# uniio/ivf-hnsw

Measured on AMD Instinct MI355X. Metric: queries/sec @ Recall@1, SIFT1B PQ16 nprobe=32; ADC scan HBM GB/s vs peak, higher is better.
Workload: dtype f32

## Files before the change

### ivf-hnsw_amd/csrc/capi_upload.cpp

```cpp
#include "capi_internal.h"

namespace {

int check_desc(const ivfhnsw_ivf_desc *d, bool need_lists)
{
    if (!d)
        return fail(IVFHNSW_ERR_INVALID, "null descriptor");
    if (d->d == 0 || d->nc == 0 || d->code_size == 0)
        return fail(IVFHNSW_ERR_INVALID, "d, nc and code_size must be positive");
    if (d->code_size % 4)
        return fail(IVFHNSW_ERR_INVALID, "code_size %zu is not a multiple of 4 (IndexIVF_HNSW.cpp:805)", d->code_size);
    if (d->code_size * 1024 > kScanDynLdsMax)
        return fail(IVFHNSW_ERR_INVALID, "code_size %zu: the query's table (1 KB per code byte) must fit %zu KB of LDS",
                    d->code_size, kScanDynLdsMax / 1024);
    if (d->d % d->code_size)
        return fail(IVFHNSW_ERR_INVALID, "d %zu is not a multiple of code_size %zu", d->d, d->code_size);
    if (d->d / d->code_size > 64)
        return fail(IVFHNSW_ERR_INVALID, "sub-vector dimension %zu > 64 unsupported", d->d / d->code_size);
    if (d->nc >= 0xffffffffull)
        return fail(IVFHNSW_ERR_INVALID, "nc too large");
    if (!d->offsets || !d->centroid_norms || !d->pq_centroids || !d->norm_table)
        return fail(IVFHNSW_ERR_INVALID, "offsets, centroid_norms, pq_centroids and norm_table are required");
    if (need_lists && d->offsets[d->nc] != 0 && (!d->ids || !d->codes || !d->norm_codes))
        return fail(IVFHNSW_ERR_INVALID, "ids, codes and norm_codes are required");
// ... 397 lines not shown
        link_counts = counts_u.data();
        links = links_u.data();
        unique = true;
    }
    if ((rc = upload(h->q_counts, link_counts, n)))
        return rc;
    if ((rc = upload(h->q_links, links, n * maxM * sizeof(uint32_t))))
        return rc;
    if ((rc = upload(h->q_vectors, vectors, n * d * sizeof(float))))
        return rc;
    h->gr.n = (uint32_t)n;
    h->gr.d = (int)d;
    h->gr.maxM = (int)maxM;
    h->gr.enterpoint = enterpoint;
    h->gr.counts = h->q_counts.as<uint8_t>();
    h->gr.links = h->q_links.as<uint32_t>();
    h->gr.vectors = h->q_vectors.as<float>();
    {
        static const int merge = [] {
            const char *e = getenv("IVFHNSW_WALK_MERGE");
            return (e && atoi(e) == 0) ? 0 : 1;
        }();
        h->gr.merge_admissions = merge;
        h->gr.skip_padding = 1;
    }
    {
        static const int late_knob = [] {
            const char *e = getenv("IVFHNSW_WALK_LATE_VISIT");
            return e ? (atoi(e) != 0 ? 1 : 0) : -1;
        }();
        const bool late = late_knob < 0 ? n > 255u * 1008u : late_knob == 1;
        h->gr.links_unique = (unique && late) ? 1 : 0;
    }
    h->gr.fat = nullptr;
    h->gr.qrows = nullptr;
    h->gr.nbrows = nullptr;
    h->gr.nbnorms = nullptr;
    h->gr.links_c = nullptr;
    h->gr.nb_rows = 0;
    h->gr.q_lo = 0.f;
    h->gr.q_step = 1.f;
    h->gr.q_errc = 0.f;
    if ((rc = build_byte_rows(h, n, d, vectors)))
        return rc;
    if ((rc = build_neighbour_rows(h)))
        return rc;
    h->has_graph = true;
// ... 96 lines not shown
```

### ivf-hnsw_amd/csrc/ivfhnsw_kernels.h

```cpp
#pragma once

#include <hip/hip_runtime.h>
#include <mutex>
#include <stdint.h>

#include "scan_dispatch.h"
#include "sweep_plan_math.h"
#include "update_math.h"

namespace ivfhnsw_gpu_impl {

struct DynLdsState {
    std::mutex m;
    size_t raised[64] = {};
};
inline hipError_t raise_dyn_lds(const void *kern, size_t bytes, DynLdsState &st)
{
    int dev = 0;
    hipError_t e = hipGetDevice(&dev);
    if (e != hipSuccess)
        return e;
    if (dev < 0 || dev >= 64)
        return hipFuncSetAttribute(kern, hipFuncAttributeMaxDynamicSharedMemorySize, (int)bytes);
    std::lock_guard<std::mutex> lk(st.m);
// ... 75 lines not shown
    int nsubc;
    const float *alphas;
    const uint32_t *nn_idx;
    const uint32_t *sub_sizes;
    const float *inter_dists;
    int dedupe;
};

struct GraphTables {
    uint32_t n;
    int d, maxM;
    uint32_t enterpoint;
    const uint8_t *counts;
    const uint32_t *links;
    const float *vectors;
    const uint8_t *qrows;
    float q_lo, q_step, q_errc;
    const uint8_t *nbrows;
    const uint32_t *nbnorms;
    const uint32_t *links_c;
    int nb_rows;
    const float *fat;
    int visited_clean;
    int skip_padding;
    int merge_admissions;
    int links_unique;
};

hipError_t launch_opq(hipStream_t s, const float *At, const float *x, float *y, int nq, int d);
hipError_t launch_lut(hipStream_t s, const IvfTables &t, const float *xq, float *luts, int nq, const PlanHdr *hdr = nullptr);
hipError_t launch_plan_ivf(hipStream_t s, const IvfTables &t, const uint32_t *coarse_ids, const float *coarse_dists,
                           int nprobe, uint64_t max_codes, const PlanView &p, uint64_t *keys, int k);
hipError_t launch_plan_lut(hipStream_t s, const IvfTables &t, const float *xq, const uint32_t *coarse_ids,
                           const float *coarse_dists, int nprobe, uint64_t max_codes, const PlanView &p, uint64_t *keys,
                           int k, float *luts);
hipError_t launch_plan_grouping(hipStream_t s, const IvfTables &t, const GroupTables &g, const GraphTables &gr,
                                const float *xq, const uint32_t *coarse_ids, const float *coarse_dists, int nprobe,
                                uint64_t max_codes, int do_pruning, const PlanView &p, uint64_t *keys, int k,
                                float *qsd_scratch);
struct ScanOut {
    uint64_t *stream = nullptr;
    uint32_t *stream_len = nullptr;
    uint32_t stream_cap = 0;
    float *sel_dist = nullptr;
    int64_t *sel_labels = nullptr;
};
hipError_t launch_scan(hipStream_t s, const IvfTables &t, const float *luts, const PlanView &p, int k, int nsplit,
// ... 194 lines not shown
```

### ivf-hnsw_amd/csrc/kernels_hnsw.hip

```cpp
#include "ivfhnsw_kernels.h"
#include "device_common.h"
#include "walk_set.h"

#include <float.h>
#include <stdio.h>
#include <stdlib.h>

namespace ivfhnsw_gpu_impl {

constexpr int vis_buckets(int minw, int tagw = 8)
{
    return minw <= 4 ? (tagw == 10 ? 1040 : 1008) : minw == 5 ? 768 : minw <= 7 ? 640 : 384;
}

template <int TAGW> struct VisFields {
    static constexpr int cntw = TAGW == 8 ? 8 : TAGW == 10 ? 14 : 16;
    static constexpr int cshift = 64 - cntw;
    static constexpr int slots = cshift / TAGW;
    static constexpr unsigned long long ones()
    {
        unsigned long long o = 0;
        for (int i = 0; i < slots; i++)
            o |= 1ull << (TAGW * i);
        return o;
    }
};

template <int TAGW, int NB>
__device__ __forceinline__ bool visit_test_and_set(uint32_t id, unsigned long long *vt, uint32_t *bm, bool &used_bitmap)
// ... 85 lines not shown
                    const float t1 = qv.y - (float)((ws[c] >> 8) & 0xffu);
                    const float t2 = qv.z - (float)((ws[c] >> 16) & 0xffu);
                    const float t3 = qv.w - (float)(ws[c] >> 24);
                    a0 = fmaf(t0, t0, a0);
                    a1 = fmaf(t1, t1, a1);
                    a2 = fmaf(t2, t2, a2);
                    a3 = fmaf(t3, t3, a3);
                }
            }
        }
    }
    return (a0 + a1) + (a2 + a3);
}

__device__ __forceinline__ unsigned long long walk_stamp()
{
    __builtin_amdgcn_sched_barrier(0);
    const unsigned long long t = __builtin_amdgcn_s_memtime();
    __builtin_amdgcn_s_waitcnt(0xC07F);
    __builtin_amdgcn_sched_barrier(0);
    return t;
}

template <int NCH, int MINW, int TAGW, int FMODE, bool STAMPS = false, bool SPILL = false>
__global__ __launch_bounds__(64, MINW) void hnsw_walk_kernel(GraphTables g, const float *__restrict__ xq, int nq, int nprobe,
                                                       int ef, uint32_t *__restrict__ coarse_ids,
                                                       float *__restrict__ coarse_dists,
                                                       uint32_t *__restrict__ visited, size_t vwords,
                                                       uint32_t *__restrict__ status, uint32_t *__restrict__ next_query,
                                                       uint32_t *__restrict__ redo_hdr, uint32_t *__restrict__ redo_list,
                                                       uint32_t *__restrict__ tail_bitmaps = nullptr,
                                                       unsigned long long *__restrict__ stamp_out = nullptr)
{
    extern __shared__ __attribute__((aligned(16))) unsigned char smem[];
    float *s_q = reinterpret_cast<float *>(smem);
    float *s_qp = s_q + g.d;
    const int dp = FMODE == 1 ? g.d : 0;
    uint32_t *s_q8 = reinterpret_cast<uint32_t *>(s_qp + dp);
    unsigned long long *tail = reinterpret_cast<unsigned long long *>(smem + (size_t)(g.d + dp) * sizeof(float) + 512);
    constexpr int NB = vis_buckets(MINW, TAGW);
    unsigned long long st_acc[9] = {0, 0, 0, 0, 0, 0}, st_t = 0;
    const int merge_extra = (NCH <= 4 && ef + 8 > kTailCap) ? ef + 8 - kTailCap : 0;
    unsigned long long *vt = tail + kTailCap + merge_extra;
    constexpr bool LDSVIS = TAGW != 0;

    const int lane = threadIdx.x;
    const int judged_row = 8 * (((lane >> 2) & 1) * 2 + (lane & 1)) + (lane >> 3);
    const bool merge_on = g.merge_admissions != 0;
    constexpr bool prefilter = FMODE != 0;
    constexpr bool inline_rows = FMODE >= 2;
    constexpr bool ROWNORMS = FMODE == 3;
    constexpr bool CK = FMODE >= 2;
    auto enc_id = [](uint32_t id, uint32_t c) { return CK ? (id << 7) | c : id; };
    auto dec_id = [](uint32_t e) { return CK ? e >> 7 : e; };
    uint32_t *bm = visited + (size_t)blockIdx.x * vwords;
    TailSpill spill;
    spill.bm = SPILL ? tail_bitmaps + (size_t)blockIdx.x * vwords : nullptr;
    spill.hi = -1;
    spill.count = 0;
    bool bitmap_dirty = !(LDSVIS && g.visited_clean);
    bool redo_ran = false;

    for (;;) {
        int q = 0;
        if constexpr (SPILL) {
            if (lane == 0) {
                const uint32_t i = atomicAdd(&redo_hdr[1], 1u);
                q = i < redo_hdr[0] ? (int)redo_list[i] : nq;
            }
        } else {
            if (lane == 0)
                q = (int)atomicAdd(next_query, 1u);
        }
        q = __builtin_amdgcn_readfirstlane(q);
        if (q >= nq)
            break;
        redo_ran = true;
        if (STAMPS)
            st_t = walk_stamp();

        if (!LDSVIS || bitmap_dirty) {
            uint4 *bm4 = reinterpret_cast<uint4 *>(bm);
            const size_t v4 = vwords / 4;
            for (size_t w = lane; w < v4; w += 64)
                bm4[w] = make_uint4(0u, 0u, 0u, 0u);
            bitmap_dirty = false;
        }
        if (LDSVIS)
            for (int w = lane; w < NB; w += 64)
                vt[w] = 0ull;
        __syncthreads();
        float qp_sq = 0.f;
        for (int i = lane; i < g.d; i += 64) {
            const float v = xq[(size_t)q * g.d + i];
            s_q[i] = v;
            if (prefilter) {
                const float vp = __fdiv_rn(__fsub_rn(v, g.q_lo), g.q_step);
                if (!inline_rows)
                    s_qp[i] = vp;
                qp_sq = fmaf(vp, vp, qp_sq);
            }
        }
        __syncthreads();
        constexpr bool QREG = MINW <= 4;
        float q_reg[QREG ? 16 : 1];
        if constexpr (QREG) {
#pragma unroll
            for (int i = 0; i < 16; i++)
                q_reg[i] = (g.d == 128 || g.d == 96) && 8 * i < g.d ? s_q[8 * i + (lane & 7)] : 0.f;
        }
        float pf_slack = 0.f, pf_slack_q = 0.f, pf_bonus = 0.f;
        int q16_w = 0;
        int x_const = 0;
        bool x_any = false;
        bool x_hi = false;
        uint4 qp_h = make_uint4(0u, 0u, 0u, 0u), qp_l = qp_h, qp_x = qp_h;
        if (prefilter) {
#pragma unroll
            for (int off = 32; off > 0; off >>= 1)
                qp_sq += __shfl_xor(qp_sq, off, 64);
            pf_slack = __uint_as_float(__builtin_amdgcn_readfirstlane(__float_as_uint(g.q_errc + 3.9e-6f * sqrtf(qp_sq))));
            if (inline_rows) {
                float dq_sq = 0.f, bonus = 0.f;
                int s_hh = 0, s_hl = 0, s_ll = 0, s_xh = 0, s_xl = 0;
                if (lane < 32) {
                    uint32_t wh = 0, wl = 0, wxl = 0, wxh = 0;
#pragma unroll
                    for (int b = 0; b < 4; b++) {
                        const int comp = 4 * lane + b;
                        const float vp = comp < g.d ? __fdiv_rn(__fsub_rn(s_q[comp], g.q_lo), g.q_step) : 0.f;
                        const float fh = fminf(255.f, fmaxf(0.f, floorf(vp)));
                        const float fl = fminf(255.f, fmaxf(0.f, rintf((vp - fh) * 256.f)));
                        const float qin = fh + fl * 0.00390625f;
                        const bool below = vp < 0.f, above = vp >= 256.f;
                        const float e = (below || above) ? 0.f : vp - qin;
                        dq_sq = fmaf(e, e, dq_sq);
                        const float out = (below || above) ? fabsf(vp - qin) : 0.f;
                        bonus = fmaf(out, out, bonus);
                        const int x = (int)fminf(255.f, floorf(2.f * out));
                        const int hi = (int)fh, lo = (int)fl;
                        s_hh += hi * hi;
                        s_hl += hi * lo;
                        s_ll += lo * lo;
                        wh |= (uint32_t)hi << (8 * b);
                        wl |= (uint32_t)lo << (8 * b);
                        if (below)
                            wxl |= (uint32_t)x << (8 * b);
                        if (above)
                            wxh |= (uint32_t)x << (8 * b);
                        s_xl += below ? x : 0;
                        s_xh += above ? x : 0;
                    }
                    s_q8[lane] = wh;
// ... 14 lines not shown
                s_xl = __builtin_amdgcn_readfirstlane(s_xl);
                s_xh = __builtin_amdgcn_readfirstlane(s_xh);
                q16_w = __builtin_amdgcn_readfirstlane(128 * s_hh + s_hl + (s_ll >> 9));
                x_any = (s_xl | s_xh) != 0;
                x_hi = s_xh != 0;
                x_const = 255 * s_xh;
                pf_slack_q = __uint_as_float(__builtin_amdgcn_readfirstlane(__float_as_uint(1.001f * sqrtf(dq_sq))));
                pf_bonus = __uint_as_float(__builtin_amdgcn_readfirstlane(__float_as_uint(0.999f * bonus)));
                __syncthreads();
                qp_h = *reinterpret_cast<const uint4 *>(s_q8 + 4 * (lane & 7));
                qp_l = *reinterpret_cast<const uint4 *>(s_q8 + 32 + 4 * (lane & 7));
                qp_x = *reinterpret_cast<const uint4 *>(s_q8 + 64 + 4 * (lane & 7));
            }
        }

        RSet<NCH> R;
#pragma unroll
        for (int cc = 0; cc < NCH; cc++)
            R.r[cc] = ~0ull;
        int n = 1;
        int ntail = 0;
        uint32_t tail_db = 0;
        {
            const float d0 = l2_ref_order_quad(g.vectors + (size_t)g.enterpoint * g.d, s_q, g.d, lane & 3);
            bool ub = false;
            if (lane == 0) {
                R.r[0] = mk_key(d0, enc_id(g.enterpoint, CK ? (uint32_t)g.counts[g.enterpoint] : 0u));
                (void)visit_test_and_set<TAGW, NB>(g.enterpoint, vt, bm, ub);
            }
            __syncthreads();
        }
        bool used_bitmap = false;
        bool pend = false, pend_any = false, pend_full = false;
        uint32_t pend_id = 0;
        if (STAMPS) {
            const unsigned long long t = walk_stamp();
            st_acc[4] += t - st_t;
            st_t = t;
        }

        for (;;) {
            const int first = R.first_unexpanded(n, lane);
            int pick = -1;
            int pick_tail = -1;
            uint32_t pick_id = 0;
            if (first >= 0) {
                const unsigned long long kfirst = R.get(first);
                const uint32_t db = key_dist_bits(kfirst);
                pick = first;
                pick_id = key_id(kfirst);
                if (first + 1 < n && key_dist_bits(R.get(first + 1)) == db) {
                    pick = R.last_unexpanded_with(db, first, n, lane);
                    pick_id = key_id(R.get(pick));
                }
                if (ntail > 0 && db == key_dist_bits(R.get(n - 1))) {
                    if (SPILL && spill.count > 0) {
                        const uint32_t sid = spill.peek_max(lane);
                        const uint32_t senc = enc_id(sid, CK ? (uint32_t)g.counts[sid] : 0u);
                        if (senc > pick_id) {
                            pick_id = senc;
                            pick_tail = kTailCap;
                        }
                    } else {
                        for (int t = 0; t < ntail; t++)
                            if (key_id(tail[t]) > pick_id) {
                                pick_id = key_id(tail[t]);
                                pick_tail = t;
                            }
                    }
                    if (pick_tail >= 0)
                        pick = -1;
                }
            } else if (SPILL && spill.count > 0) {
                const uint32_t sid = spill.peek_max(lane);
                pick_id = enc_id(sid, CK ? (uint32_t)g.counts[sid] : 0u);
                pick_tail = kTailCap;
            } else if (ntail > 0) {
                pick_tail = 0;
                pick_id = key_id(tail[0]);
                for (int t = 1; t < ntail; t++)
                    if (key_id(tail[t]) > pick_id) {
                        pick_id = key_id(tail[t]);
                        pick_tail = t;
                    }
            } else {
                break;
            }
            if (pick >= 0) {
                R.mark_expanded(pick, lane);
            } else if (SPILL && pick_tail == kTailCap) {
                spill.remove(dec_id(pick_id), lane);
                ntail--;
            } else {
                __syncthreads();
                if (lane == 0)
                    tail[pick_tail] = tail[ntail - 1];
                ntail--;
                __syncthreads();
            }

            if (STAMPS) {
                const unsigned long long t = walk_stamp();
                st_acc[0] += t - st_t;
                st_t = t;
                st_acc[5] += 1;
            }
            const uint32_t node = dec_id(pick_id);
            int cnt;
            uint32_t nb = 0, nb_enc = 0;
            if constexpr (CK) {
                cnt = (int)(pick_id & 127u);
                if (lane < g.maxM) {
                    const uint32_t raw = g.links_c[(size_t)node * g.maxM + lane];
                    nb = raw & 0xffffffu;
                    nb_enc = (nb << 7) | (raw >> 24);
                }
            } else {
                cnt = g.counts[node];
                if (lane < g.maxM)
                    nb = g.links[(size_t)node * g.maxM + lane];
                nb_enc = nb;
            }
            const bool filter_now = prefilter && n == ef;
            uint4 nw[4] = {};
            uint32_t row_rr = 0;
            if (filter_now && inline_rows) {
                if constexpr (CK) {
                    const uint4 *nbr = reinterpret_cast<const uint4 *>(g.nbrows + (size_t)node * g.nb_rows * 128) + (lane & 7);
                    const int last = max(cnt - 1, 0);
#pragma unroll
                    for (int i = 0; i < 4; i++)
                        if (8 * i < cnt)
                            nw[i] = nbr[min(8 * i + (lane >> 3), last) * 8];
                } else {
                    const uint4 *nbr = reinterpret_cast<const uint4 *>(g.nbrows + (size_t)node * g.nb_rows * 128) + lane;
#pragma unroll
                    for (int i = 0; i < 4; i++)
                        nw[i] = nbr[i * 64];
                }
                if constexpr (ROWNORMS)
                    row_rr = g.nbnorms[(size_t)node * g.nb_rows + judged_row];
            }
            constexpr bool LATE = FMODE == 3 && LDSVIS;
            const bool filter_first = LATE && filter_now;
            bool fresh = false, seen = false, full_now = false;
            if constexpr (LATE) {
                if (pend_any) {
                    if (pend)
                        visit_insert_absent<TAGW, NB>(pend_id, pend_full, vt, bm, used_bitmap);
                    pend_any = false;
                }
                if (lane < cnt) {
                    if (filter_first)
                        seen = visit_lookup<TAGW, NB>(nb, vt, bm, full_now);
                    else
                        fresh = visit_test_and_set<TAGW, NB>(nb, vt, bm, used_bitmap);
                }
            } else {
                if (lane < cnt)
                    fresh = visit_test_and_set<TAGW, NB>(nb, vt, bm, used_bitmap);
            }
            unsigned long long mask = __ballot(fresh);
            int nfresh = __popcll(mask);
            const unsigned long long last_now = R.get(n - 1);
            if (filter_now && inline_rows) {
                if (filter_first)
                    fresh = lane < cnt && !seen;
                const float worst = __uint_as_float(key_dist_bits(last_now));
                const uint32_t qh[4] = {qp_h.x, qp_h.y, qp_h.z, qp_h.w}, ql[4] = {qp_l.x, qp_l.y, qp_l.z, qp_l.w};
                const uint32_t xl[4] = {qp_x.x, qp_x.y, qp_x.z, qp_x.w};
                uint32_t xh[4] = {0u, 0u, 0u, 0u};
                if (x_hi) {
                    const uint4 b = *reinterpret_cast<const uint4 *>(s_q8 + 96 + 4 * (lane & 7));
                    xh[0] = b.x, xh[1] = b.y, xh[2] = b.z, xh[3] = b.w;
                }
                const int cnt_s = __builtin_amdgcn_readfirstlane(cnt);
                for (int rb = 0;;) {
                    int S[4], X[4];
#pragma unroll
                    for (int i = 0; i < 4; i++) {
                        if ((CK || g.skip_padding) && rb + 8 * i >= cnt_s) {
                            S[i] = 0;
                            X[i] = 0;
                            continue;
                        }
                        const uint32_t ws[4] = {nw[i].x, nw[i].y, nw[i].z, nw[i].w};
                        uint32_t hr = 0, rr = 0;
#pragma unroll
                        for (int c = 0; c < 4; c++) {
                            hr = __builtin_amdgcn_udot4(qh[c], ws[c], hr, false);
                            if constexpr (!ROWNORMS)
                                rr = __builtin_amdgcn_udot4(ws[c], ws[c], rr, false);
                        }
                        uint32_t lr = hr << 8;
#pragma unroll
                        for (int c = 0; c < 4; c++)
                            lr = __builtin_amdgcn_udot4(ql[c], ws[c], lr, false);
                        S[i] = (int)(128u * rr - lr);
                        X[i] = 0;
                        if (x_any) {
                            uint32_t xlr = 0, xhr = 0;
#pragma unroll
                            for (int c = 0; c < 4; c++)
                                xlr = __builtin_amdgcn_udot4(xl[c], ws[c], xlr, false);
// ... 7 lines not shown
                        }
                    }
                    int mine, minex = 0;
                    if (x_any)
                        oct_sum4x2(S, X, lane, mine, minex);
                    else
                        mine = oct_sum4(S, lane);
                    mine += (int)(128u * row_rr);
                    const float m1 = fmaxf(
                        0.f, __builtin_amdgcn_sqrtf((float)(mine + q16_w) * 0.0078125f) * 0.9990234375f - pf_slack_q);
                    const float m2 = fmaf(m1, m1, fmaf((float)(minex + x_const), 0.9990234375f, pf_bonus));
                    const float m = fmaxf(0.f, __builtin_amdgcn_sqrtf(m2) * 0.9990234375f - pf_slack) * g.q_step;
                    const float lb = m * m * 0.9990234375f;
                    const unsigned long long dropm = __ballot(lb > worst) & 0x3333333333333333ull;
                    const int rel = lane - rb;
                    const int ri = rel >> 3;
                    if (rel >= 0 && rel < 32 && ((dropm >> (8 * (rel & 7) + 4 * (ri >> 1) + (ri & 1))) & 1ull))
                        fresh = false;
                    rb += 32;
                    if (rb >= cnt)
                        break;
                    if constexpr (CK) {
                        const uint4 *nbr =
                            reinterpret_cast<const uint4 *>(g.nbrows + (size_t)node * g.nb_rows * 128) + (lane & 7);
                        const int last = max(cnt - 1, 0);
#pragma unroll
                        for (int i = 0; i < 4; i++)
                            if (rb + 8 * i < cnt)
                                nw[i] = nbr[min(rb + 8 * i + (lane >> 3), last) * 8];
                    } else {
                        const uint4 *nbr =
                            reinterpret_cast<const uint4 *>(g.nbrows + ((size_t)node * g.nb_rows + rb) * 128) + lane;
#pragma unroll
                        for (int i = 0; i < 4; i++)
                            nw[i] = nbr[i * 64];
                    }
                    if constexpr (ROWNORMS)
                        row_rr = g.nbnorms[(size_t)node * g.nb_rows + rb + judged_row];
                }
                mask = __ballot(fresh);
                nfresh = __popcll(mask);
                if (filter_first) {
                    pend = fresh;
                    pend_full = full_now;
                    pend_id = nb;
                    pend_any = nfresh > 0;
                }
            } else if (filter_now && nfresh > 0) {
                const float worst = __uint_as_float(key_dist_bits(last_now));
                const int myrow = __popcll(mask & ((1ull << lane) - 1ull));
                for (int base = 0; base < nfresh; base += 32) {
                    const int r = base + (lane >> 1);
                    const bool active = r < nfresh;
                    const int src = active ? nth_set_bit(mask, r) : 0;
                    const uint32_t nbq = (uint32_t)__shfl((int)nb, src, 64);
                    float S = 0.f;
                    if (active)
                        S = byte_row_dist_half(g.qrows + (size_t)nbq * g.d, s_qp, g.d, lane & 1);
                    S += __shfl_xor(S, 1, 64);
                    const float m = fmaxf(0.f, __builtin_amdgcn_sqrtf(S) * 0.9990234375f - pf_slack) * g.q_step;
                    const float lb = m * m * 0.9990234375f;
                    const unsigned long long drop = __ballot(active && lb > worst);
                    const int rel = myrow - base;
                    if (fresh && rel >= 0 && rel < 32 && ((drop >> (2 * rel)) & 1ull))
                        fresh = false;
                }
                mask = __ballot(fresh);
                nfresh = __popcll(mask);
            }
            if (STAMPS) {
                const unsigned long long t = walk_stamp();
                st_acc[1] += t - st_t;
                st_t = t;
            }

            unsigned long long rest = mask;
            for (int base = 0; base < nfresh && ntail >= 0; base += 8) {
                const int r = base + (lane >> 3);
                const bool active = r < nfresh;
                const int src = take8_set_bits(rest, lane);
                const uint32_t nbe = (uint32_t)__shfl((int)nb_enc, src, 64);
                const uint32_t nbq = dec_id(nbe);
                float dq = 0.f;
                if (active) {
                    if constexpr (QREG)
                        dq = g.d == 128  ? l2_ref_order_oct_regs<16>(g.vectors + (size_t)nbq * 128, q_reg, lane & 7)
                             : g.d == 96 ? l2_ref_order_oct_regs<12>(g.vectors + (size_t)nbq * 96, q_reg, lane & 7)
                                         : l2_ref_order_oct(g.vectors + (size_t)nbq * g.d, s_q, g.d, lane & 7);
                    else
                        dq = l2_ref_order_oct(g.vectors + (size_t)nbq * g.d, s_q, g.d, lane & 7);
                }
                if (STAMPS) {
                    asm volatile("s_waitcnt vmcnt(0)" ::: "memory");
                    const unsigned long long t = walk_stamp();
                    st_acc[2] += t - st_t;
                    st_t = t;
                }
                unsigned long long topk = base == 0 ? last_now : R.get(n - 1);
                const float top0 = __uint_as_float(key_dist_bits(topk));
                unsigned long long cand = (n < ef ? ~0ull : __ballot(top0 > dq)) & 0x0101010101010101ull &
                                          lanes_below(8 * (nfresh - base), 0);
                if (STAMPS) {
                    st_acc[6] += (unsigned long long)__popcll(__ballot(active && (lane & 7) == 0));
                    st_acc[7] += (unsigned long long)__popcll(cand);
                }
                if (NCH <= 4 && merge_on && n == ef && ntail == 0 && cand) {
                    const bool is_cand = (cand >> lane) & 1ull;
                    const unsigned long long Kc = mk_key(dq, nbe);
                    int dn[NCH];
#pragma unroll
                    for (int cc = 0; cc < NCH; cc++)
                        dn[cc] = 0;
                    const int ncand = __popcll(cand);
                    int cand_below = 0, set_below = 0;
                    for (unsigned long long cm = cand; cm; cm &= cm - 1) {
                        const int b = __ffsll((long long)cm) - 1;
                        const unsigned long long Kj = readlane_u64(Kc, b);
                        int below = 0;
#pragma unroll
                        for (int cc = 0; cc < NCH; cc++) {
                            const bool lt = (R.r[cc] & ~1ull) < Kj;
                            below += __popcll(__ballot(lt) & lanes_below(ef, cc));
                            dn[cc] += lt ? 1 : 0;
                        }
                        cand_below += Kj < Kc ? 1 : 0;
                        set_below = lane == b ? below : set_below;
                    }
                    unsigned long long *mb = tail;
#pragma unroll
// ... 5 lines not shown
                    __syncthreads();
                    const unsigned long long b_lo = mb[ef - 1], b_hi = mb[ef];
                    unsigned long long merged[NCH];
#pragma unroll
                    for (int cc = 0; cc < NCH; cc++)
                        merged[cc] = cc * 64 + lane < ef ? mb[cc * 64 + lane] : R.r[cc];
                    const bool clean = key_dist_bits(b_lo) != key_dist_bits(b_hi);
                    if (clean) {
#pragma unroll
                        for (int cc = 0; cc < NCH; cc++)
                            R.r[cc] = merged[cc];
                        if (STAMPS)
                            st_acc[8] += (unsigned long long)__popcll(__ballot(is_cand && set_below + cand_below < ef));
                        cand = 0;
                    }
                    __syncthreads();
                }
                while (cand) {
                    const int b = __ffsll((long long)cand) - 1;
                    cand &= cand - 1;
                    const float dj = __uint_as_float((uint32_t)__builtin_amdgcn_readlane((int)__float_as_uint(dq), b));
                    const uint32_t idj = (uint32_t)__builtin_amdgcn_readlane((int)nbe, b);
                    const unsigned long long oldtop = topk;
                    if (!(__uint_as_float(key_dist_bits(oldtop)) > dj || n < ef))
                        continue;
                    const unsigned long long K = mk_key(dj, idj);
                    const bool full = n == ef;
                    if (STAMPS)
                        st_acc[8] += 1;
                    R.insert_sorted(K, lane);
                    if (!full)
                        n++;
                    topk = R.get(n - 1);
                    const uint32_t newmax = key_dist_bits(topk);
                    if (ntail > 0 && (SPILL ? tail_db : key_dist_bits(tail[0])) != newmax) {
                        ntail = 0;
                        if (SPILL && spill.count > 0)
                            spill.clear(lane);
                    }
                    if (full && !(oldtop & 1ull) && key_dist_bits(oldtop) == newmax) {
                        if (SPILL)
                            tail_db = newmax;
                        if ((!SPILL || spill.count == 0) && ntail < kTailCap) {
                            __syncthreads();
                            if (lane == 0)
                                tail[ntail] = oldtop;
                            ntail++;
                            __syncthreads();
                        } else if constexpr (SPILL) {
                            if (spill.count == 0) {
                                __syncthreads();
                                for (int t = 0; t < ntail; t++)
                                    spill.add(dec_id(key_id(tail[t])), lane);
                                __syncthreads();
                            }
                            spill.add(dec_id(key_id(oldtop)), lane);
                            ntail++;
                        } else {
                            if (lane == 0)
                                redo_list[atomicAdd(&redo_hdr[0], 1u)] = (uint32_t)q;
                            ntail = -1;
                            break;
                        }
                    }
                }
                if (STAMPS) {
                    const unsigned long long t = walk_stamp();
                    st_acc[3] += t - st_t;
                    st_t = t;
                }
            }
            if (ntail < 0)
                break;
        }

        if (SPILL && spill.count > 0)
            spill.clear(lane);
        if (LDSVIS && __ballot(used_bitmap))
            bitmap_dirty = true;
        if (ntail >= 0) {
#pragma unroll
            for (int cc = 0; cc < NCH; cc++) {
                const int i = cc * 64 + lane;
                if (i < nprobe) {
                    const bool have = i < n;
                    coarse_ids[(size_t)q * nprobe + i] = have ? dec_id(key_id(R.r[cc])) : 0xffffffffu;
                    coarse_dists[(size_t)q * nprobe + i] = have ? __uint_as_float(key_dist_bits(R.r[cc])) : 0.f;
                }
            }
        }
    }
    if constexpr (SPILL) {
        if (lane == 0) {
            __threadfence();
            if (atomicAdd(&redo_hdr[2], 1u) == gridDim.x - 1) {
                redo_hdr[-1] = 0;
                redo_hdr[0] = 0;
                redo_hdr[1] = 0;
                redo_hdr[2] = 0;
            }
        }
    }
    if (SPILL && redo_ran) {
        uint4 *bm4 = reinterpret_cast<uint4 *>(bm);
        for (size_t w = lane; w < vwords / 4; w += 64)
            bm4[w] = make_uint4(0u, 0u, 0u, 0u);
    }
    if (LDSVIS && bitmap_dirty) {
        uint4 *bm4 = reinterpret_cast<uint4 *>(bm);
        for (size_t w = lane; w < vwords / 4; w += 64)
            bm4[w] = make_uint4(0u, 0u, 0u, 0u);
    }
    if (STAMPS && stamp_out && lane == 0)
        for (int i = 0; i < 9; i++)
            atomicAdd(&stamp_out[i], st_acc[i]);
}

__global__ __launch_bounds__(64) void build_nbrows_kernel(GraphTables g, uint8_t *__restrict__ nbrows,
                                                          uint32_t *__restrict__ nbnorms, int nb_rows,
                                                          uint32_t *__restrict__ links_c)
{
    const size_t node = blockIdx.x;
    const int cnt = g.counts[node];
    if ((int)threadIdx.x < g.maxM) {
        uint32_t e = 0;
        if ((int)threadIdx.x < cnt) {
            const uint32_t id = g.links[node * g.maxM + threadIdx.x];
            e = id | ((uint32_t)g.counts[id] << 24);
        }
        links_c[node * g.maxM + threadIdx.x] = e;
    }
    const int cpr = g.d >> 4;
    for (int r0 = 0; r0 < nb_rows; r0 += 8) {
        const int r = r0 + (threadIdx.x >> 3), c = threadIdx.x & 7;
        uint4 v = make_uint4(0u, 0u, 0u, 0u);
        if (r < cnt && c < cpr)
            v = reinterpret_cast<const uint4 *>(g.qrows + (size_t)g.links[node * g.maxM + r] * g.d)[c];
        reinterpret_cast<uint4 *>(nbrows + (node * nb_rows + r) * 128)[c] = v;
// ... 64 lines not shown
    if ((tagw == 12 || tagw == 10) && occ_eff == 4 && g.n <= 1023u * (uint32_t)vis_buckets(4, 10) && force_tagw != 12) {
        tagw = 10;
        nbk = (uint32_t)vis_buckets(4, 10);
    } else if (tagw == 10) {
        tagw = 12;
    }
    const size_t shm = (size_t)(g.d + ((g.qrows && !g.nbrows) ? g.d : 0)) * sizeof(float) + 512 +
                       (size_t)(kTailCap + ((ef <= 256 && ef + 8 > kTailCap) ? ef + 8 - kTailCap : 0)) *
                           sizeof(unsigned long long) +
                       (tagw ? (size_t)nbk * sizeof(unsigned long long) : 0);
    const int fmode = g.nbrows ? (g.links_unique && tagw ? 3 : 2) : g.qrows ? 1 : 0;
    g.visited_clean = 0;
    if (tagw && visited_zero) {
        if (!*visited_zero) {
            e = hipMemsetAsync(visited_scratch, 0, visited_bytes, s);
            if (e != hipSuccess)
                return e;
        }
        g.visited_clean = 1;
        *visited_zero = true;
    } else if (visited_zero) {
        *visited_zero = false;
    }
#define IVFHNSW_WALK_F(N, W, T, F)                                                                                    \
    hipLaunchKernelGGL((hnsw_walk_kernel<N, W, T, F>), dim3(nslots), dim3(64), shm, s, g, xq, nq, nprobe, ef,         \
                       coarse_ids, coarse_dists, visited_scratch, visited_words_per_slot, status, next_query, redo_hdr, redo_list)
#define IVFHNSW_WALK_T(N, W, T)          \
    do {                                 \
        if (fmode == 3)                  \
            IVFHNSW_WALK_F(N, W, T, 3);  \
        else if (fmode == 2)             \
            IVFHNSW_WALK_F(N, W, T, 2);  \
        else if (fmode == 1)             \
            IVFHNSW_WALK_F(N, 4, T, 1);  \
        else                             \
            IVFHNSW_WALK_F(N, 4, T, 0);  \
    } while (0)
#define IVFHNSW_WALK(N, W)             \
    do {                               \
        if (tagw == 8)                 \
            IVFHNSW_WALK_T(N, W, 8);   \
        else if (tagw == 10)           \
            IVFHNSW_WALK_T(N, 4, 10);  \
        else if (tagw == 12)           \
            IVFHNSW_WALK_T(N, W, 12);  \
        else if (tagw == 16)           \
            IVFHNSW_WALK_T(N, W, 16);  \
        else                           \
            IVFHNSW_WALK_T(N, W, 0);   \
    } while (0)
#define IVFHNSW_WALK_N(N) IVFHNSW_WALK(N, 4)
    static const bool stamps = [] {
        const char *e = getenv("IVFHNSW_WALK_STAMPS");
        return e && atoi(e) == 1;
    }();
    if (stamps && nch == 2 && ((tagw == 8 && fmode == 2) || (tagw == 10 && fmode == 3)) && occ == 4) {
        static unsigned long long *d_st = nullptr;
        if (!d_st) {
            (void)hipMalloc(&d_st, 9 * sizeof(unsigned long long));
            (void)hipMemset(d_st, 0, 9 * sizeof(unsigned long long));
            atexit([] {
                unsigned long long h[9];
                if (hipMemcpy(h, d_st, sizeof(h), hipMemcpyDeviceToHost) == hipSuccess) {
                    const double tot = (double)(h[0] + h[1] + h[2] + h[3] + h[4]);
                    fprintf(stderr, "[walk stamps] expansions %llu; cycles/expansion: select %.0f, links+visited %.0f, "
                                    "distances %.0f, admissions %.0f; prologue share %.1f%%; total wave-cycles %.3g\n",
                            h[5], (double)h[0] / h[5], (double)h[1] / h[5], (double)h[2] / h[5], (double)h[3] / h[5],
                            100.0 * h[4] / tot, tot);
                    fprintf(stderr, "[walk stamps] rows evaluated/expansion %.2f, passing the wave-wide test %.2f, admitted %.2f\n",
                            (double)h[6] / h[5], (double)h[7] / h[5], (double)h[8] / h[5]);
                }
            });
        }
        if (tagw == 8)
            hipLaunchKernelGGL((hnsw_walk_kernel<2, 4, 8, 2, true>), dim3(nslots), dim3(64), shm, s, g, xq, nq, nprobe, ef,
                               coarse_ids, coarse_dists, visited_scratch, visited_words_per_slot, status, next_query, redo_hdr,
                               redo_list, nullptr, d_st);
        else
            hipLaunchKernelGGL((hnsw_walk_kernel<2, 4, 10, 3, true>), dim3(nslots), dim3(64), shm, s, g, xq, nq, nprobe, ef,
                               coarse_ids, coarse_dists, visited_scratch, visited_words_per_slot, status, next_query, redo_hdr,
                               redo_list, nullptr, d_st);
        return hipGetLastError();
    }
    if (nch <= 1) {
        IVFHNSW_WALK_N(1);
    } else if (nch <= 2) {
        IVFHNSW_WALK_N(2);
    } else if (nch == 3) {
        IVFHNSW_WALK_N(3);
    } else if (nch <= 4) {
        IVFHNSW_WALK_N(4);
    } else if (nch <= 8) {
        IVFHNSW_WALK(8, 4);
    } else {
        IVFHNSW_WALK(16, 4);
    }
#undef IVFHNSW_WALK_N
#undef IVFHNSW_WALK
#undef IVFHNSW_WALK_T
#undef IVFHNSW_WALK_F
    e = hipGetLastError();
    if (e != hipSuccess)
        return e;
    e = launch_coarse_redo(s, g, xq, nq, nprobe, ef, coarse_ids, coarse_dists, visited_scratch, visited_words_per_slot,
                           status, redo_hdr, redo_list, tail_bitmaps, tail_slots);
    if (e == hipSuccess && counters_clean)
        *counters_clean = true;
    return e;
}

hipError_t launch_coarse_redo(hipStream_t s, const GraphTables &g_in, const float *xq, int nq, int nprobe, int ef,
                              uint32_t *coarse_ids, float *coarse_dists, uint32_t *visited_scratch,
                              size_t visited_words_per_slot, uint32_t *status, uint32_t *redo_hdr, uint32_t *redo_list,
                              uint32_t *tail_bitmaps, int tail_slots)
{
    GraphTables g = g_in;
    g.visited_clean = 0;
    const int nch = (ef + 63) / 64;
    const int slots = std::min(std::min(nq, tail_slots), 64);
    const size_t shm = (size_t)g.d * sizeof(float) + 512 +
                       (size_t)(kTailCap + ((ef <= 256 && ef + 8 > kTailCap) ? ef + 8 - kTailCap : 0)) * sizeof(unsigned long long);
#define IVFHNSW_REDO(N)                                                                                               \
    hipLaunchKernelGGL((hnsw_walk_kernel<N, 4, 0, 0, false, true>), dim3(slots), dim3(64), shm, s, g, xq, nq, nprobe, ef, \
                       coarse_ids, coarse_dists, visited_scratch, visited_words_per_slot, status, redo_hdr + 1, redo_hdr, \
                       redo_list, tail_bitmaps)
    if (nch <= 1)
        IVFHNSW_REDO(1);
    else if (nch <= 2)
        IVFHNSW_REDO(2);
    else if (nch == 3)
        IVFHNSW_REDO(3);
    else if (nch <= 4)
        IVFHNSW_REDO(4);
    else if (nch <= 8)
        IVFHNSW_REDO(8);
    else
        IVFHNSW_REDO(16);
#undef IVFHNSW_REDO
    return hipGetLastError();
}

}
```

Before: 6.144 million.

## Specialize HNSW walk kernel on compile-time dimension and degree, split warmup/steady phases

Adds template parameters for vector dimension, maxM and merge mode so common shapes (d=128/96, maxM=32) get constant-folded addressing and distance loops. The main expansion loop becomes a lambda instantiated separately for the fill phase and the steady phase, where the set size equals ef. Kernel arguments are packed into a struct, and rarely used fields are re-read late from the kernarg segment to cut SGPR pressure. The skip_padding flag is removed and padding is always skipped. The cost is many more kernel instantiations and larger code size.

```diff
diff --git a/ivf-hnsw_amd/csrc/capi_upload.cpp b/ivf-hnsw_amd/csrc/capi_upload.cpp
--- a/ivf-hnsw_amd/csrc/capi_upload.cpp
+++ b/ivf-hnsw_amd/csrc/capi_upload.cpp
@@ -443,7 +443,6 @@
             return (e && atoi(e) == 0) ? 0 : 1;
         }();
         h->gr.merge_admissions = merge;
-        h->gr.skip_padding = 1;
     }
     {
         static const int late_knob = [] {
diff --git a/ivf-hnsw_amd/csrc/ivfhnsw_kernels.h b/ivf-hnsw_amd/csrc/ivfhnsw_kernels.h
--- a/ivf-hnsw_amd/csrc/ivfhnsw_kernels.h
+++ b/ivf-hnsw_amd/csrc/ivfhnsw_kernels.h
@@ -121,7 +121,6 @@
     int nb_rows;
     const float *fat;
     int visited_clean;
-    int skip_padding;
     int merge_admissions;
     int links_unique;
 };
diff --git a/ivf-hnsw_amd/csrc/kernels_hnsw.hip b/ivf-hnsw_amd/csrc/kernels_hnsw.hip
--- a/ivf-hnsw_amd/csrc/kernels_hnsw.hip
+++ b/ivf-hnsw_amd/csrc/kernels_hnsw.hip
@@ -1,10 +1,12 @@
 #include "ivfhnsw_kernels.h"
 #include "device_common.h"
 #include "walk_set.h"
+#include "walk_shape.h"
 
 #include <float.h>
 #include <stdio.h>
 #include <stdlib.h>
+#include <type_traits>
 
 namespace ivfhnsw_gpu_impl {
 
@@ -136,22 +138,49 @@
     return t;
 }
 
-template <int NCH, int MINW, int TAGW, int FMODE, bool STAMPS = false, bool SPILL = false>
-__global__ __launch_bounds__(64, MINW) void hnsw_walk_kernel(GraphTables g, const float *__restrict__ xq, int nq, int nprobe,
-                                                       int ef, uint32_t *__restrict__ coarse_ids,
-                                                       float *__restrict__ coarse_dists,
-                                                       uint32_t *__restrict__ visited, size_t vwords,
-                                                       uint32_t *__restrict__ status, uint32_t *__restrict__ next_query,
-                                                       uint32_t *__restrict__ redo_hdr, uint32_t *__restrict__ redo_list,
-                                                       uint32_t *__restrict__ tail_bitmaps = nullptr,
-                                                       unsigned long long *__restrict__ stamp_out = nullptr)
-{
+
+struct WalkArgs {
+    GraphTables g;
+    const float *xq;
+    int nq, nprobe, ef;
+    uint32_t *coarse_ids;
+    float *coarse_dists;
+    uint32_t *visited;
+    size_t vwords;
+    uint32_t *status, *next_query, *redo_hdr, *redo_list;
+    uint32_t *tail_bitmaps;
+    unsigned long long *stamp_out;
+};
+
+template <class T> __device__ __forceinline__ const __attribute__((address_space(4))) T *late_kernarg()
+{
+    auto p = (const __attribute__((address_space(4))) T *)__builtin_amdgcn_kernarg_segment_ptr();
+    asm volatile("" : "+s"(p));
+    return p;
+}
+
+template <int NCH, int MINW, int TAGW, int FMODE, bool STAMPS = false, bool SPILL = false, int D = 0, int MAXM = 0,
+          bool MERGE = true>
+__global__ __launch_bounds__(64, MINW) void hnsw_walk_kernel(WalkArgs a)
+{
+    constexpr bool SHAPED = D != 0 && MAXM != 0;
+    const GraphTables &g = a.g;
+    const int ef = a.ef;
+    uint32_t *__restrict__ const visited = a.visited;
+    const size_t vwords = a.vwords;
+#define WALK_COLD(f) (SHAPED ? late_kernarg<WalkArgs>()->f : a.f)
     extern __shared__ __attribute__((aligned(16))) unsigned char smem[];
     float *s_q = reinterpret_cast<float *>(smem);
-    float *s_qp = s_q + g.d;
-    const int dp = FMODE == 1 ? g.d : 0;
+    static_assert(!SHAPED || (FMODE >= 2 && !SPILL && MINW <= 4 && D % 16 == 0 && D <= 128 && MAXM <= 64),
+                  "shape constants go with the neighbour-row forms");
+    static_assert(SHAPED || MERGE, "the generic form reads merge_admissions at run time");
+    const int dim = D ? D : g.d;
+    const int maxm = MAXM ? MAXM : g.maxM;
+    const int nbr_rows = MAXM ? (MAXM + 31) / 32 * 32 : g.nb_rows;
+    float *s_qp = s_q + dim;
+    const int dp = FMODE == 1 ? dim : 0;
     uint32_t *s_q8 = reinterpret_cast<uint32_t *>(s_qp + dp);
-    unsigned long long *tail = reinterpret_cast<unsigned long long *>(smem + (size_t)(g.d + dp) * sizeof(float) + 512);
+    unsigned long long *tail = reinterpret_cast<unsigned long long *>(smem + (size_t)(dim + dp) * sizeof(float) + 512);
     constexpr int NB = vis_buckets(MINW, TAGW);
     unsigned long long st_acc[9] = {0, 0, 0, 0, 0, 0}, st_t = 0;
     const int merge_extra = (NCH <= 4 && ef + 8 > kTailCap) ? ef + 8 - kTailCap : 0;
@@ -160,7 +189,7 @@
 
     const int lane = threadIdx.x;
     const int judged_row = 8 * (((lane >> 2) & 1) * 2 + (lane & 1)) + (lane >> 3);
-    const bool merge_on = g.merge_admissions != 0;
+    const bool merge_on = SHAPED ? MERGE : g.merge_admissions != 0;
     constexpr bool prefilter = FMODE != 0;
     constexpr bool inline_rows = FMODE >= 2;
     constexpr bool ROWNORMS = FMODE == 3;
@@ -169,7 +198,7 @@
     auto dec_id = [](uint32_t e) { return CK ? e >> 7 : e; };
     uint32_t *bm = visited + (size_t)blockIdx.x * vwords;
     TailSpill spill;
-    spill.bm = SPILL ? tail_bitmaps + (size_t)blockIdx.x * vwords : nullptr;
+    spill.bm = SPILL ? a.tail_bitmaps + (size_t)blockIdx.x * vwords : nullptr;
     spill.hi = -1;
     spill.count = 0;
     bool bitmap_dirty = !(LDSVIS && g.visited_clean);
@@ -179,15 +208,15 @@
         int q = 0;
         if constexpr (SPILL) {
             if (lane == 0) {
-                const uint32_t i = atomicAdd(&redo_hdr[1], 1u);
-                q = i < redo_hdr[0] ? (int)redo_list[i] : nq;
+                const uint32_t i = atomicAdd(&a.redo_hdr[1], 1u);
+                q = i < a.redo_hdr[0] ? (int)a.redo_list[i] : a.nq;
             }
         } else {
             if (lane == 0)
-                q = (int)atomicAdd(next_query, 1u);
+                q = (int)atomicAdd(WALK_COLD(next_query), 1u);
         }
         q = __builtin_amdgcn_readfirstlane(q);
-        if (q >= nq)
+        if (q >= WALK_COLD(nq))
             break;
         redo_ran = true;
         if (STAMPS)
@@ -205,11 +234,11 @@
                 vt[w] = 0ull;
         __syncthreads();
         float qp_sq = 0.f;
-        for (int i = lane; i < g.d; i += 64) {
-            const float v = xq[(size_t)q * g.d + i];
+        for (int i = lane; i < dim; i += 64) {
+            const float v = WALK_COLD(xq)[(size_t)q * dim + i];
             s_q[i] = v;
             if (prefilter) {
-                const float vp = __fdiv_rn(__fsub_rn(v, g.q_lo), g.q_step);
+                const float vp = __fdiv_rn(__fsub_rn(v, WALK_COLD(g.q_lo)), g.q_step);
                 if (!inline_rows)
                     s_qp[i] = vp;
                 qp_sq = fmaf(vp, vp, qp_sq);
@@ -221,7 +250,10 @@
         if constexpr (QREG) {
 #pragma unroll
             for (int i = 0; i < 16; i++)
-                q_reg[i] = (g.d == 128 || g.d == 96) && 8 * i < g.d ? s_q[8 * i + (lane & 7)] : 0.f;
+                if constexpr (D != 0)
+                    q_reg[i] = 8 * i < D ? s_q[8 * i + (lane & 7)] : 0.f;
+                else
+                    q_reg[i] = (g.d == 128 || g.d == 96) && 8 * i < g.d ? s_q[8 * i + (lane & 7)] : 0.f;
         }
         float pf_slack = 0.f, pf_slack_q = 0.f, pf_bonus = 0.f;
         int q16_w = 0;
@@ -233,7 +265,7 @@
 #pragma unroll
             for (int off = 32; off > 0; off >>= 1)
                 qp_sq += __shfl_xor(qp_sq, off, 64);
-            pf_slack = __uint_as_float(__builtin_amdgcn_readfirstlane(__float_as_uint(g.q_errc + 3.9e-6f * sqrtf(qp_sq))));
+            pf_slack = __uint_as_float(__builtin_amdgcn_readfirstlane(__float_as_uint(WALK_COLD(g.q_errc) + 3.9e-6f * sqrtf(qp_sq))));
             if (inline_rows) {
                 float dq_sq = 0.f, bonus = 0.f;
                 int s_hh = 0, s_hl = 0, s_ll = 0, s_xh = 0, s_xl = 0;
@@ -242,7 +274,7 @@
 #pragma unroll
                     for (int b = 0; b < 4; b++) {
                         const int comp = 4 * lane + b;
-                        const float vp = comp < g.d ? __fdiv_rn(__fsub_rn(s_q[comp], g.q_lo), g.q_step) : 0.f;
+                        const float vp = comp < dim ? __fdiv_rn(__fsub_rn(s_q[comp], WALK_COLD(g.q_lo)), g.q_step) : 0.f;
                         const float fh = fminf(255.f, fmaxf(0.f, floorf(vp)));
                         const float fl = fminf(255.f, fmaxf(0.f, rintf((vp - fh) * 256.f)));
                         const float qin = fh + fl * 0.00390625f;
@@ -303,11 +335,12 @@
         int ntail = 0;
         uint32_t tail_db = 0;
         {
-            const float d0 = l2_ref_order_quad(g.vectors + (size_t)g.enterpoint * g.d, s_q, g.d, lane & 3);
+            const uint32_t ep = WALK_COLD(g.enterpoint);
+            const float d0 = l2_ref_order_quad(g.vectors + (size_t)ep * dim, s_q, dim, lane & 3);
             bool ub = false;
             if (lane == 0) {
-                R.r[0] = mk_key(d0, enc_id(g.enterpoint, CK ? (uint32_t)g.counts[g.enterpoint] : 0u));
-                (void)visit_test_and_set<TAGW, NB>(g.enterpoint, vt, bm, ub);
+                R.r[0] = mk_key(d0, enc_id(ep, CK ? (uint32_t)WALK_COLD(g.counts)[ep] : 0u));
+                (void)visit_test_and_set<TAGW, NB>(ep, vt, bm, ub);
             }
             __syncthreads();
         }
@@ -320,8 +353,11 @@
             st_t = t;
         }
 
-        for (;;) {
-            const int first = R.first_unexpanded(n, lane);
+        auto expand = [&](auto phase_c) __attribute__((always_inline)) -> bool {
+            constexpr int PHASE = decltype(phase_c)::value;
+            constexpr bool STEADY = PHASE == 2;
+            auto set_n = [&] { return STEADY ? ef : n; };
+            const int first = R.first_unexpanded(set_n(), lane);
             int pick = -1;
             int pick_tail = -1;
             uint32_t pick_id = 0;
@@ -330,11 +366,11 @@
                 const uint32_t db = key_dist_bits(kfirst);
                 pick = first;
                 pick_id = key_id(kfirst);
-                if (first + 1 < n && key_dist_bits(R.get(first + 1)) == db) {
-                    pick = R.last_unexpanded_with(db, first, n, lane);
+                if (first + 1 < set_n() && key_dist_bits(R.get(first + 1)) == db) {
+                    pick = R.last_unexpanded_with(db, first, set_n(), lane);
                     pick_id = key_id(R.get(pick));
                 }
-                if (ntail > 0 && db == key_dist_bits(R.get(n - 1))) {
+                if (ntail > 0 && db == key_dist_bits(R.get(set_n() - 1))) {
                     if (SPILL && spill.count > 0) {
                         const uint32_t sid = spill.peek_max(lane);
                         const uint32_t senc = enc_id(sid, CK ? (uint32_t)g.counts[sid] : 0u);
@@ -365,7 +401,7 @@
                         pick_tail = t;
                     }
             } else {
-                break;
+                return false;
             }
             if (pick >= 0) {
                 R.mark_expanded(pick, lane);
@@ -391,42 +427,42 @@
             uint32_t nb = 0, nb_enc = 0;
             if constexpr (CK) {
                 cnt = (int)(pick_id & 127u);
-                if (lane < g.maxM) {
-                    const uint32_t raw = g.links_c[(size_t)node * g.maxM + lane];
+                if (lane < maxm) {
+                    const uint32_t raw = g.links_c[(size_t)node * maxm + lane];
                     nb = raw & 0xffffffu;
                     nb_enc = (nb << 7) | (raw >> 24);
                 }
             } else {
                 cnt = g.counts[node];
-                if (lane < g.maxM)
-                    nb = g.links[(size_t)node * g.maxM + lane];
+                if (lane < maxm)
+                    nb = g.links[(size_t)node * maxm + lane];
                 nb_enc = nb;
             }
-            const bool filter_now = prefilter && n == ef;
+            const bool filter_now = PHASE == 0 ? prefilter && n == ef : prefilter && STEADY;
             uint4 nw[4] = {};
             uint32_t row_rr = 0;
             if (filter_now && inline_rows) {
                 if constexpr (CK) {
-                    const uint4 *nbr = reinterpret_cast<const uint4 *>(g.nbrows + (size_t)node * g.nb_rows * 128) + (lane & 7);
+                    const uint4 *nbr = reinterpret_cast<const uint4 *>(g.nbrows + (size_t)node * nbr_rows * 128) + (lane & 7);
                     const int last = max(cnt - 1, 0);
 #pragma unroll
                     for (int i = 0; i < 4; i++)
                         if (8 * i < cnt)
                             nw[i] = nbr[min(8 * i + (lane >> 3), last) * 8];
                 } else {
-                    const uint4 *nbr = reinterpret_cast<const uint4 *>(g.nbrows + (size_t)node * g.nb_rows * 128) + lane;
+                    const uint4 *nbr = reinterpret_cast<const uint4 *>(g.nbrows + (size_t)node * nbr_rows * 128) + lane;
 #pragma unroll
                     for (int i = 0; i < 4; i++)
                         nw[i] = nbr[i * 64];
                 }
                 if constexpr (ROWNORMS)
-                    row_rr = g.nbnorms[(size_t)node * g.nb_rows + judged_row];
+                    row_rr = g.nbnorms[(size_t)node * nbr_rows + judged_row];
             }
             constexpr bool LATE = FMODE == 3 && LDSVIS;
             const bool filter_first = LATE && filter_now;
             bool fresh = false, seen = false, full_now = false;
             if constexpr (LATE) {
-                if (pend_any) {
+                if (PHASE != 1 && pend_any) {
                     if (pend)
                         visit_insert_absent<TAGW, NB>(pend_id, pend_full, vt, bm, used_bitmap);
                     pend_any = false;
@@ -443,7 +479,7 @@
             }
             unsigned long long mask = __ballot(fresh);
             int nfresh = __popcll(mask);
-            const unsigned long long last_now = R.get(n - 1);
+            const unsigned long long last_now = R.get(set_n() - 1);
             if (filter_now && inline_rows) {
                 if (filter_first)
                     fresh = lane < cnt && !seen;
@@ -460,7 +496,7 @@
                     int S[4], X[4];
 #pragma unroll
                     for (int i = 0; i < 4; i++) {
-                        if ((CK || g.skip_padding) && rb + 8 * i >= cnt_s) {
+                        if (rb + 8 * i >= cnt_s) {
                             S[i] = 0;
                             X[i] = 0;
                             continue;
@@ -514,7 +550,7 @@
                         break;
                     if constexpr (CK) {
                         const uint4 *nbr =
-                            reinterpret_cast<const uint4 *>(g.nbrows + (size_t)node * g.nb_rows * 128) + (lane & 7);
+                            reinterpret_cast<const uint4 *>(g.nbrows + (size_t)node * nbr_rows * 128) + (lane & 7);
                         const int last = max(cnt - 1, 0);
 #pragma unroll
                         for (int i = 0; i < 4; i++)
@@ -522,13 +558,13 @@
                                 nw[i] = nbr[min(rb + 8 * i + (lane >> 3), last) * 8];
                     } else {
                         const uint4 *nbr =
-                            reinterpret_cast<const uint4 *>(g.nbrows + ((size_t)node * g.nb_rows + rb) * 128) + lane;
+                            reinterpret_cast<const uint4 *>(g.nbrows + ((size_t)node * nbr_rows + rb) * 128) + lane;
 #pragma unroll
                         for (int i = 0; i < 4; i++)
                             nw[i] = nbr[i * 64];
                     }
                     if constexpr (ROWNORMS)
-                        row_rr = g.nbnorms[(size_t)node * g.nb_rows + rb + judged_row];
+                        row_rr = g.nbnorms[(size_t)node * nbr_rows + rb + judged_row];
                 }
                 mask = __ballot(fresh);
                 nfresh = __popcll(mask);
@@ -548,7 +584,7 @@
                     const uint32_t nbq = (uint32_t)__shfl((int)nb, src, 64);
                     float S = 0.f;
                     if (active)
-                        S = byte_row_dist_half(g.qrows + (size_t)nbq * g.d, s_qp, g.d, lane & 1);
+                        S = byte_row_dist_half(g.qrows + (size_t)nbq * dim, s_qp, dim, lane & 1);
                     S += __shfl_xor(S, 1, 64);
                     const float m = fmaxf(0.f, __builtin_amdgcn_sqrtf(S) * 0.9990234375f - pf_slack) * g.q_step;
                     const float lb = m * m * 0.9990234375f;
@@ -575,7 +611,9 @@
                 const uint32_t nbq = dec_id(nbe);
                 float dq = 0.f;
                 if (active) {
-                    if constexpr (QREG)
+                    if constexpr (D != 0)
+                        dq = l2_ref_order_oct_regs<D / 8>(g.vectors + (size_t)nbq * D, q_reg, lane & 7);
+                    else if constexpr (QREG)
                         dq = g.d == 128  ? l2_ref_order_oct_regs<16>(g.vectors + (size_t)nbq * 128, q_reg, lane & 7)
                              : g.d == 96 ? l2_ref_order_oct_regs<12>(g.vectors + (size_t)nbq * 96, q_reg, lane & 7)
                                          : l2_ref_order_oct(g.vectors + (size_t)nbq * g.d, s_q, g.d, lane & 7);
@@ -588,15 +626,15 @@
                     st_acc[2] += t - st_t;
                     st_t = t;
                 }
-                unsigned long long topk = base == 0 ? last_now : R.get(n - 1);
+                unsigned long long topk = base == 0 ? last_now : R.get(set_n() - 1);
                 const float top0 = __uint_as_float(key_dist_bits(topk));
-                unsigned long long cand = (n < ef ? ~0ull : __ballot(top0 > dq)) & 0x0101010101010101ull &
+                unsigned long long cand = (!STEADY && n < ef ? ~0ull : __ballot(top0 > dq)) & 0x0101010101010101ull &
                                           lanes_below(8 * (nfresh - base), 0);
                 if (STAMPS) {
                     st_acc[6] += (unsigned long long)__popcll(__ballot(active && (lane & 7) == 0));
                     st_acc[7] += (unsigned long long)__popcll(cand);
                 }
-                if (NCH <= 4 && merge_on && n == ef && ntail == 0 && cand) {
+                if (NCH <= 4 && merge_on && (STEADY || n == ef) && ntail == 0 && cand) {
                     const bool is_cand = (cand >> lane) & 1ull;
                     const unsigned long long Kc = mk_key(dq, nbe);
                     int dn[NCH];
@@ -648,16 +686,16 @@
                     const float dj = __uint_as_float((uint32_t)__builtin_amdgcn_readlane((int)__float_as_uint(dq), b));
                     const uint32_t idj = (uint32_t)__builtin_amdgcn_readlane((int)nbe, b);
                     const unsigned long long oldtop = topk;
-                    if (!(__uint_as_float(key_dist_bits(oldtop)) > dj || n < ef))
+                    if (!(__uint_as_float(key_dist_bits(oldtop)) > dj || (!STEADY && n < ef)))
                         continue;
                     const unsigned long long K = mk_key(dj, idj);
-                    const bool full = n == ef;
+                    const bool full = STEADY || n == ef;
                     if (STAMPS)
                         st_acc[8] += 1;
                     R.insert_sorted(K, lane);
                     if (!full)
                         n++;
-                    topk = R.get(n - 1);
+                    topk = R.get(set_n() - 1);
                     const uint32_t newmax = key_dist_bits(topk);
                     if (ntail > 0 && (SPILL ? tail_db : key_dist_bits(tail[0])) != newmax) {
                         ntail = 0;
@@ -684,7 +722,7 @@
                             ntail++;
                         } else {
                             if (lane == 0)
-                                redo_list[atomicAdd(&redo_hdr[0], 1u)] = (uint32_t)q;
+                                WALK_COLD(redo_list)[atomicAdd(&WALK_COLD(redo_hdr)[0], 1u)] = (uint32_t)q;
                             ntail = -1;
                             break;
                         }
@@ -696,8 +734,17 @@
                     st_t = t;
                 }
             }
-            if (ntail < 0)
-                break;
+            return ntail >= 0;
+        };
+        if constexpr (SHAPED) {
+            bool live = true;
+            while (live && n < ef)
+                live = expand(std::integral_constant<int, 1>{});
+            while (live)
+                live = expand(std::integral_constant<int, 2>{});
+        } else {
+            while (expand(std::integral_constant<int, 0>{})) {
+            }
         }
 
         if (SPILL && spill.count > 0)
@@ -708,10 +755,11 @@
 #pragma unroll
             for (int cc = 0; cc < NCH; cc++) {
                 const int i = cc * 64 + lane;
+                const int nprobe = WALK_COLD(nprobe);
                 if (i < nprobe) {
                     const bool have = i < n;
-                    coarse_ids[(size_t)q * nprobe + i] = have ? dec_id(key_id(R.r[cc])) : 0xffffffffu;
-                    coarse_dists[(size_t)q * nprobe + i] = have ? __uint_as_float(key_dist_bits(R.r[cc])) : 0.f;
+                    WALK_COLD(coarse_ids)[(size_t)q * nprobe + i] = have ? dec_id(key_id(R.r[cc])) : 0xffffffffu;
+                    WALK_COLD(coarse_dists)[(size_t)q * nprobe + i] = have ? __uint_as_float(key_dist_bits(R.r[cc])) : 0.f;
                 }
             }
         }
@@ -719,11 +767,11 @@
     if constexpr (SPILL) {
         if (lane == 0) {
             __threadfence();
-            if (atomicAdd(&redo_hdr[2], 1u) == gridDim.x - 1) {
-                redo_hdr[-1] = 0;
-                redo_hdr[0] = 0;
-                redo_hdr[1] = 0;
-                redo_hdr[2] = 0;
+            if (atomicAdd(&a.redo_hdr[2], 1u) == gridDim.x - 1) {
+                a.redo_hdr[-1] = 0;
+                a.redo_hdr[0] = 0;
+                a.redo_hdr[1] = 0;
+                a.redo_hdr[2] = 0;
             }
         }
     }
@@ -737,9 +785,10 @@
         for (size_t w = lane; w < vwords / 4; w += 64)
             bm4[w] = make_uint4(0u, 0u, 0u, 0u);
     }
-    if (STAMPS && stamp_out && lane == 0)
+    if (STAMPS && a.stamp_out && lane == 0)
         for (int i = 0; i < 9; i++)
-            atomicAdd(&stamp_out[i], st_acc[i]);
+            atomicAdd(&a.stamp_out[i], st_acc[i]);
+#undef WALK_COLD
 }
 
 __global__ __launch_bounds__(64) void build_nbrows_kernel(GraphTables g, uint8_t *__restrict__ nbrows,
@@ -850,9 +899,9 @@
     } else if (visited_zero) {
         *visited_zero = false;
     }
-#define IVFHNSW_WALK_F(N, W, T, F)                                                                                    \
-    hipLaunchKernelGGL((hnsw_walk_kernel<N, W, T, F>), dim3(nslots), dim3(64), shm, s, g, xq, nq, nprobe, ef,         \
-                       coarse_ids, coarse_dists, visited_scratch, visited_words_per_slot, status, next_query, redo_hdr, redo_list)
+    WalkArgs wa = {g,      xq,         nq,       nprobe,    ef,      coarse_ids, coarse_dists, visited_scratch, visited_words_per_slot,
+                   status, next_query, redo_hdr, redo_list, nullptr, nullptr};
+#define IVFHNSW_WALK_F(N, W, T, F) hipLaunchKernelGGL((hnsw_walk_kernel<N, W, T, F>), dim3(nslots), dim3(64), shm, s, wa)
 #define IVFHNSW_WALK_T(N, W, T)          \
     do {                                 \
         if (fmode == 3)                  \
@@ -882,6 +931,12 @@
         const char *e = getenv("IVFHNSW_WALK_STAMPS");
         return e && atoi(e) == 1;
     }();
+    static const bool shape_on = [] {
+        const char *e = getenv("IVFHNSW_WALK_SHAPE");
+        return !(e && atoi(e) == 0);
+    }();
+    const WalkShape shape = walk_shape_for(g.d, g.maxM, g.nb_rows, fmode, tagw, nch, shape_on);
+    const bool merge = g.merge_admissions != 0;
     if (stamps && nch == 2 && ((tagw == 8 && fmode == 2) || (tagw == 10 && fmode == 3)) && occ == 4) {
         static unsigned long long *d_st = nullptr;
         if (!d_st) {
@@ -900,16 +955,51 @@
                 }
             });
         }
+        wa.stamp_out = d_st;
         if (tagw == 8)
-            hipLaunchKernelGGL((hnsw_walk_kernel<2, 4, 8, 2, true>), dim3(nslots), dim3(64), shm, s, g, xq, nq, nprobe, ef,
-                               coarse_ids, coarse_dists, visited_scratch, visited_words_per_slot, status, next_query, redo_hdr,
-                               redo_list, nullptr, d_st);
+            hipLaunchKernelGGL((hnsw_walk_kernel<2, 4, 8, 2, true>), dim3(nslots), dim3(64), shm, s, wa);
+        else if (shape.d == 128 && merge)
+            hipLaunchKernelGGL((hnsw_walk_kernel<2, 4, 10, 3, true, false, 128, 32, true>), dim3(nslots), dim3(64), shm, s, wa);
         else
-            hipLaunchKernelGGL((hnsw_walk_kernel<2, 4, 10, 3, true>), dim3(nslots), dim3(64), shm, s, g, xq, nq, nprobe, ef,
-                               coarse_ids, coarse_dists, visited_scratch, visited_words_per_slot, status, next_query, redo_hdr,
-                               redo_list, nullptr, d_st);
+            hipLaunchKernelGGL((hnsw_walk_kernel<2, 4, 10, 3, true>), dim3(nslots), dim3(64), shm, s, wa);
         return hipGetLastError();
     }
+#define IVFHNSW_WALK_S(N, T, F, DD, MG) \
+    hipLaunchKernelGGL((hnsw_walk_kernel<N, 4, T, F, false, false, DD, 32, MG>), dim3(nslots), dim3(64), shm, s, wa)
+#define IVFHNSW_WALK_SD(N, T, F)                   \
+    do {                                           \
+        if (shape.d == 128 && merge)               \
+            IVFHNSW_WALK_S(N, T, F, 128, true);    \
+        else if (shape.d == 128)                   \
+            IVFHNSW_WALK_S(N, T, F, 128, false);   \
+        else if (merge)                            \
+            IVFHNSW_WALK_S(N, T, F, 96, true);     \
+        else                                       \
+            IVFHNSW_WALK_S(N, T, F, 96, false);    \
+    } while (0)
+#define IVFHNSW_WALK_ST(N, T)            \
+    do {                                 \
+        if (fmode == 3)                  \
+            IVFHNSW_WALK_SD(N, T, 3);    \
+        else                             \
+            IVFHNSW_WALK_SD(N, T, 2);    \
+    } while (0)
+#define IVFHNSW_WALK_SN(N)               \
+    do {                                 \
+        if (tagw == 8)                   \
+            IVFHNSW_WALK_ST(N, 8);       \
+        else if (tagw == 10)             \
+            IVFHNSW_WALK_ST(N, 10);      \
+        else if (tagw == 12)             \
+            IVFHNSW_WALK_ST(N, 12);      \
+        else                             \
+            IVFHNSW_WALK_ST(N, 16);      \
+    } while (0)
+    if (shape.d != 0 && nch <= 1) {
+        IVFHNSW_WALK_SN(1);
+    } else if (shape.d != 0) {
+        IVFHNSW_WALK_SN(2);
+    } else
     if (nch <= 1) {
         IVFHNSW_WALK_N(1);
     } else if (nch <= 2) {
@@ -923,6 +1013,10 @@
     } else {
         IVFHNSW_WALK(16, 4);
     }
+#undef IVFHNSW_WALK_SN
+#undef IVFHNSW_WALK_ST
+#undef IVFHNSW_WALK_SD
+#undef IVFHNSW_WALK_S
 #undef IVFHNSW_WALK_N
 #undef IVFHNSW_WALK
 #undef IVFHNSW_WALK_T
@@ -948,10 +1042,9 @@
     const int slots = std::min(std::min(nq, tail_slots), 64);
     const size_t shm = (size_t)g.d * sizeof(float) + 512 +
                        (size_t)(kTailCap + ((ef <= 256 && ef + 8 > kTailCap) ? ef + 8 - kTailCap : 0)) * sizeof(unsigned long long);
-#define IVFHNSW_REDO(N)                                                                                               \
-    hipLaunchKernelGGL((hnsw_walk_kernel<N, 4, 0, 0, false, true>), dim3(slots), dim3(64), shm, s, g, xq, nq, nprobe, ef, \
-                       coarse_ids, coarse_dists, visited_scratch, visited_words_per_slot, status, redo_hdr + 1, redo_hdr, \
-                       redo_list, tail_bitmaps)
+    const WalkArgs wa = {g,      xq,           nq,       nprobe,    ef,           coarse_ids, coarse_dists, visited_scratch, visited_words_per_slot,
+                         status, redo_hdr + 1, redo_hdr, redo_list, tail_bitmaps, nullptr};
+#define IVFHNSW_REDO(N) hipLaunchKernelGGL((hnsw_walk_kernel<N, 4, 0, 0, false, true>), dim3(slots), dim3(64), shm, s, wa)
     if (nch <= 1)
         IVFHNSW_REDO(1);
     else if (nch <= 2)
diff --git a/ivf-hnsw_amd/csrc/walk_shape.h b/ivf-hnsw_amd/csrc/walk_shape.h
--- /dev/null
+++ b/ivf-hnsw_amd/csrc/walk_shape.h
@@ -0,0 +1,21 @@
+#pragma once
+
+namespace ivfhnsw_gpu_impl {
+
+struct WalkShape {
+    int d;
+    int maxM;
+};
+
+inline WalkShape walk_shape_for(int d, int maxM, int nb_rows, int fmode, int tagw, int nch, bool shape_on)
+{
+    const WalkShape generic = {0, 0};
+    if (!shape_on || (fmode != 2 && fmode != 3) || tagw == 0 || nch < 1 || nch > 2)
+        return generic;
+    if (maxM != 32 || nb_rows != 32 || (d != 128 && d != 96))
+        return generic;
+    const WalkShape s = {d, 32};
+    return s;
+}
+
+}
```

Measured after the change: 6.440 million, median of 6. 4.8% higher.
